# Wu-sm/Adversarial-Attacks-on-GAN-based-Image-Fusion

Hardware: AMD Instinct MI355X
Metric: attacked images/sec, PGD-20 L∞ ε=8/255 at 256², 1/2/4/8 MI355X (higher is better)
Workload: dtype f32; 1 GPU; PGD-20 L∞ eps=8/255 alpha=2/255 at 256², 128 images/GPU (BASELINE config #4 per-GPU share), RCCL all-gather of outputs when N>1; encoder=e4e, norm=linf, images_per_gpu=128, global_batch=128, size=256, pgd_steps=20, parallelism=dp1, dist_world_size=1, output_in_eps_ball_and_finite=True, fp32_arithmetic=fp32

## Files before the change

### adversarial-attacks-on-gan-based-image-fusion_amd/csrc/conv_common.h

```cpp
#pragma once
#include <algorithm>
#include <cstdlib>
#include <type_traits>

#include "mia_common.h"

namespace mia {

struct ConvGroup {
  const void* w;
  int kpad, kh, kw, pad_y, pad_x, ho, wo, ay, by, ax, bx, blk0, nbm, m;
  const void* w_split;
  int n_in, n_out, c_off;
};
constexpr int MIA_MAX_GROUPS = 16;

inline int pixels_clamped(int n, int h, int w) {
  const int64_t m = (int64_t)n * h * w;
  return m < 0 ? -1 : (m > 0x7fffffff ? 0x7fffffff : (int)m);
}

struct ConvK {
  mia_conv_args a;
  int stride, HT, WT, ystride, cout_mod, log2cin, n_first_max, ng, nblk, nbn;
// ... 338 lines not shown
            if (single) part[e] += c;
            else red_put(k, 0, pix, n * Cout + col + e, c);
          }
        }
        if (Y) {
          const size_t off = ((size_t)(n * k.HT + yo) * k.WT + xo) * k.ystride + cm;
          if (p.out_scale) {
            if (!single) load8f(p.out_scale + (size_t)n * k.cout_mod + cm, osc8);
#pragma unroll
            for (int e = 0; e < 8; ++e) v[e] *= osc8[e];
          }
          if (p.noise) {
            const float nz = p.noise_w * p.noise[yo * k.WT + xo];
#pragma unroll
            for (int e = 0; e < 8; ++e) v[e] += nz;
          }
          if (p.bias) {
#pragma unroll
            for (int e = 0; e < 8; ++e) v[e] += bias8[e];
          }
          float ma[8];
          if (TA) {
            float tt[8];
            load8<T>(TA + aoff, ma);
            load8<T>(TT + aoff, tt);
#pragma unroll
            for (int e = 0; e < 8; ++e) v[e] += p.tap_coef * (ma[e] - tt[e]);
          }
          if (MA) {
            if (MA != TA) load8<T>(MA + aoff, ma);
#pragma unroll
            for (int e = 0; e < 8; ++e) v[e] = ma[e] > 0.f ? v[e] : mslope8[e] * v[e];
          }
          if (prelu) {
#pragma unroll
            for (int e = 0; e < 8; ++e) v[e] = v[e] > 0.f ? v[e] : aslope8[e] * v[e];
          } else {
#pragma unroll
            for (int e = 0; e < 8; ++e) v[e] = apply_act(v[e], p.act_out);
          }
          if (p.accumulate) {
            float yo8[8];
            load8<T>(Y + off, yo8);
#pragma unroll
            for (int e = 0; e < 8; ++e) v[e] += yo8[e];
          }
          if (bab) {
            float dm8[8];
            load8f(p.bab_demod + (size_t)n * Cout + col, dm8);
            const float nz = p.bab_noise ? p.bab_noise_w * p.bab_noise[yo * k.WT + xo] : 0.f;
#pragma unroll
            for (int e = 0; e < 8; ++e) {
              const float gr = lrelu_s2_grad(xv[e]);
              const float gp = v[e] * gr;
              const float c = gp * (xv[e] * lrelu_s2_inv_grad(xv[e]) - nz - bbias8[e]);
              if (single) partq[e] += c;
              else red_put(k, 1, pix, n * Cout + col + e, c);
              v[e] = gp * dm8[e];
            }
          }
          if (p.csum) {
#pragma unroll
            for (int e = 0; e < 8; ++e) {
              if (single) pcs[e] += v[e];
              else red_put(k, 2, pix, n * Cout + col + e, v[e]);
            }
          }
          store8<T>(Y + off, v);
        }
      }
    }
    __syncthreads();
  }

  if (bab && single) {
#pragma unroll
    for (int e = 0; e < 8; ++e)
      for (int o = CPR; o < 64; o <<= 1) partq[e] += __shfl_xor(partq[e], o, 64);
    float* red = (float*)smem;
    if (worker && lane < CPR) {
#pragma unroll
      for (int e = 0; e < 8; ++e) red[wid * BN + lane * 8 + e] = partq[e];
    }
    __syncthreads();
    if (tid < BN && n0 + tid < Cout) {
      float s = 0.f;
#pragma unroll
      for (int w = 0; w < NW; ++w) s += red[w * BN + tid];
      red_put(k, 1, slot, n_single * Cout + n0 + tid, s);
    }
    __syncthreads();
  }
  if (p.csum && single) {
#pragma unroll
    for (int e = 0; e < 8; ++e)
      for (int o = CPR; o < 64; o <<= 1) pcs[e] += __shfl_xor(pcs[e], o, 64);
    float* red = (float*)smem;
    if (worker && lane < CPR) {
#pragma unroll
      for (int e = 0; e < 8; ++e) red[wid * BN + lane * 8 + e] = pcs[e];
    }
    __syncthreads();
    if (tid < BN && n0 + tid < Cout) {
      float s = 0.f;
#pragma unroll
      for (int w = 0; w < NW; ++w) s += red[w * BN + tid];
      red_put(k, 2, slot, n_single * Cout + n0 + tid, s);
    }
    __syncthreads();
  }
  if (p.sdot && single) {
#pragma unroll
    for (int e = 0; e < 8; ++e)
      for (int o = CPR; o < 64; o <<= 1) part[e] += __shfl_xor(part[e], o, 64);
    float* red = (float*)smem;
    if (worker && lane < CPR) {
#pragma unroll
      for (int e = 0; e < 8; ++e) red[wid * BN + lane * 8 + e] = part[e];
    }
    __syncthreads();
    if (tid < BN && n0 + tid < Cout) {
      float s = 0.f;
#pragma unroll
      for (int w = 0; w < NW; ++w) s += red[w * BN + tid];
      red_put(k, 0, slot, n_single * Cout + n0 + tid, s);
    }
  }
}

__device__ __forceinline__ void wait_vmcnt(int n) {
  switch (n) {
    case 0: asm volatile("s_waitcnt vmcnt(0)" ::: "memory"); break;
    case 1: asm volatile("s_waitcnt vmcnt(1)" ::: "memory"); break;
    case 2: asm volatile("s_waitcnt vmcnt(2)" ::: "memory"); break;
    case 3: asm volatile("s_waitcnt vmcnt(3)" ::: "memory"); break;
    case 4: asm volatile("s_waitcnt vmcnt(4)" ::: "memory"); break;
    case 5: asm volatile("s_waitcnt vmcnt(5)" ::: "memory"); break;
    case 6: asm volatile("s_waitcnt vmcnt(6)" ::: "memory"); break;
    case 7: asm volatile("s_waitcnt vmcnt(7)" ::: "memory"); break;
    case 8: asm volatile("s_waitcnt vmcnt(8)" ::: "memory"); break;
    case 9: asm volatile("s_waitcnt vmcnt(9)" ::: "memory"); break;
    case 10: asm volatile("s_waitcnt vmcnt(10)" ::: "memory"); break;
    case 11: asm volatile("s_waitcnt vmcnt(11)" ::: "memory"); break;
    case 12: asm volatile("s_waitcnt vmcnt(12)" ::: "memory"); break;
    case 13: asm volatile("s_waitcnt vmcnt(13)" ::: "memory"); break;
    case 14: asm volatile("s_waitcnt vmcnt(14)" ::: "memory"); break;
    case 15: asm volatile("s_waitcnt vmcnt(15)" ::: "memory"); break;
    default: asm volatile("s_waitcnt vmcnt(16)" ::: "memory"); break;
  }
}

bool conv_halo_x6_eligible(const ConvK& k, int dtype);
int launch_conv_halo_x6(ConvK& k, hipStream_t st);
bool conv_halo_eligible(const ConvK& k, int dtype);
int launch_conv_halo(ConvK& k, int dtype, hipStream_t st);
bool upconv_halo_eligible(int dtype, int R, int Cin, int Cout);
int launch_upconv_halo(const void* x, const void* w_up, const void* w_up_split, void* t, int N,
                       int R, int Cin, int Cout, int act_in, const float* style, int dtype,
                       hipStream_t st);
bool conv_wres_eligible(const ConvK& k, int dtype);
int launch_conv_wres(ConvK& k, int dtype, hipStream_t st);
bool conv_wres128_eligible(const ConvK& k, int dtype);
int launch_conv_wres128(ConvK& k, int dtype, hipStream_t st);
bool conv_wres32_eligible(const ConvK& k, int dtype);
int launch_conv_wres32(ConvK& k, int dtype, hipStream_t st);
bool conv_thin_eligible(const ConvK& k, int dtype);
bool conv_thin32_eligible(const ConvK& k, int dtype);
int launch_conv_thin32(ConvK& k, int dtype, hipStream_t st);
int launch_conv_thin(ConvK& k, int dtype, hipStream_t st);

}
```

### adversarial-attacks-on-gan-based-image-fusion_amd/csrc/conv_mfma.hip

```cpp
#include "conv_common.h"
#include <cstdio>
#include "halo_epilogue.h"

#ifndef MIA_F32_PRO_SMALLTILE
#define MIA_F32_PRO_SMALLTILE 128
#endif

namespace mia {

template <int PER>
__device__ __forceinline__ void wait_dma_steps(int steps) {
  static_assert(3 * PER <= 63, "vmcnt field");
  if (steps <= 0) asm volatile("s_waitcnt vmcnt(0)" ::: "memory");
  else if (steps == 1) asm volatile("s_waitcnt vmcnt(%0)" ::"n"(PER) : "memory");
  else if (steps == 2) asm volatile("s_waitcnt vmcnt(%0)" ::"n"(2 * PER) : "memory");
  else asm volatile("s_waitcnt vmcnt(%0)" ::"n"(3 * PER) : "memory");
}

template <typename T, int BM, int BN, bool X6B>
struct StageBytes {
  static constexpr int v = (BM + BN) * ROWB;
};
template <int BM, int BN>
struct StageBytes<float, BM, BN, true> {
// ... 311 lines not shown
    return -1;
  using namespace epi;
  const int f = epi_mask(k);
  switch (f) {
    case OSC | SDOT: case OSC | SDOT | ACC: case OSC | SDOT | BAB: case OSC | SDOT | ACC | BAB:
    case BIAS | PRELU:
    case BIAS: case ACC: case BIAS | ACC:
      return f;
    default:
      return -1;
  }
}

template <typename T, bool PRO, bool SMALLC>
static int launch_bn(ConvK& k, hipStream_t st) {
  int64_t m = 0;
  for (int g = 0; g < k.ng; ++g) m += k.g[g].m;
  if (k.a.Cout <= 64) {
    if constexpr (!PRO) {
      using namespace epi;
      switch (reg_epi_mask(k, sizeof(T))) {
        case OSC | SDOT: return launch_tile<T, Tile128x64, PRO, SMALLC, OSC | SDOT>(k, st);
        case OSC | SDOT | ACC:
          return launch_tile<T, Tile128x64, PRO, SMALLC, OSC | SDOT | ACC>(k, st);
        case OSC | SDOT | BAB:
          return launch_tile<T, Tile128x64, PRO, SMALLC, OSC | SDOT | BAB>(k, st);
        case OSC | SDOT | ACC | BAB:
          return launch_tile<T, Tile128x64, PRO, SMALLC, OSC | SDOT | ACC | BAB>(k, st);
        case BIAS | PRELU: return launch_tile<T, Tile128x64, PRO, SMALLC, BIAS | PRELU>(k, st);
        case BIAS: return launch_tile<T, Tile128x64, PRO, SMALLC, BIAS>(k, st);
        case ACC: return launch_tile<T, Tile128x64, PRO, SMALLC, ACC>(k, st);
        case BIAS | ACC: return launch_tile<T, Tile128x64, PRO, SMALLC, BIAS | ACC>(k, st);
        default: break;
      }
    }
    return launch_tile<T, Tile128x64, PRO, SMALLC>(k, st);
  }
  int64_t tiles = 0;
  for (int g = 0; g < k.ng; ++g) tiles += (k.g[g].m + 127) / 128;
  tiles *= (k.a.Cout + 127) / 128;
  const int64_t small_below = tune(T_CONV_SMALLTILE);
  if (sizeof(T) == 2 && tiles < small_below) return launch_tile<T, Tile64x64, PRO, SMALLC>(k, st);
  if (sizeof(T) == 4 && PRO && tiles < MIA_F32_PRO_SMALLTILE)
    return launch_tile<T, Tile64x64, PRO, SMALLC>(k, st);
  if constexpr (!SMALLC && !PRO) {
    using namespace epi;
    switch (reg_epi_mask(k, sizeof(T))) {
      case OSC | SDOT: return launch_tile<T, Tile128x128, PRO, SMALLC, OSC | SDOT>(k, st);
      case OSC | SDOT | ACC: return launch_tile<T, Tile128x128, PRO, SMALLC, OSC | SDOT | ACC>(k, st);
      case OSC | SDOT | BAB: return launch_tile<T, Tile128x128, PRO, SMALLC, OSC | SDOT | BAB>(k, st);
      case OSC | SDOT | ACC | BAB:
        return launch_tile<T, Tile128x128, PRO, SMALLC, OSC | SDOT | ACC | BAB>(k, st);
      case BIAS | PRELU: return launch_tile<T, Tile128x128, PRO, SMALLC, BIAS | PRELU>(k, st);
      case BIAS: return launch_tile<T, Tile128x128, PRO, SMALLC, BIAS>(k, st);
      case ACC: return launch_tile<T, Tile128x128, PRO, SMALLC, ACC>(k, st);
      case BIAS | ACC: return launch_tile<T, Tile128x128, PRO, SMALLC, BIAS | ACC>(k, st);
      default: break;
    }
  }
  return launch_tile<T, Tile128x128, PRO, SMALLC>(k, st);
}

static bool x6b_ok(const ConvK& k) {
#ifdef MIA_F32_NATIVE
  (void)k;
  return false;
#else
  if (tune(T_CONV_X6) == 0) return false;
  for (int g = 0; g < k.ng; ++g)
    if (!k.g[g].w_split) return false;
  return k.a.in_scale == nullptr && k.a.act_in == MIA_ACT_NONE && k.a.Cin >= 32 && k.a.Cout > 64;
#endif
}

template <typename T>
static int launch_conv(ConvK& k, hipStream_t st) {
  if constexpr (std::is_same<T, float>::value) {
    if (x6b_ok(k)) {
      using namespace epi;
      switch (reg_epi_mask(k, 4)) {
        case OSC | SDOT: return launch_tile<T, Tile128x128, false, false, OSC | SDOT, true>(k, st);
        case OSC | SDOT | ACC:
          return launch_tile<T, Tile128x128, false, false, OSC | SDOT | ACC, true>(k, st);
        case OSC | SDOT | BAB:
          return launch_tile<T, Tile128x128, false, false, OSC | SDOT | BAB, true>(k, st);
        case OSC | SDOT | ACC | BAB:
          return launch_tile<T, Tile128x128, false, false, OSC | SDOT | ACC | BAB, true>(k, st);
        case BIAS | PRELU: return launch_tile<T, Tile128x128, false, false, BIAS | PRELU, true>(k, st);
        case BIAS: return launch_tile<T, Tile128x128, false, false, BIAS, true>(k, st);
        case ACC: return launch_tile<T, Tile128x128, false, false, ACC, true>(k, st);
        case BIAS | ACC: return launch_tile<T, Tile128x128, false, false, BIAS | ACC, true>(k, st);
        default: break;
      }
      return launch_tile<T, Tile128x128, false, false, -2, true>(k, st);
    }
  }
  const bool pro = k.a.in_scale != nullptr || k.a.act_in != MIA_ACT_NONE;
  const bool small = k.a.Cin < ROWB / (int)sizeof(T);
  if (pro) return small ? launch_bn<T, true, true>(k, st) : launch_bn<T, true, false>(k, st);
  return small ? launch_bn<T, false, true>(k, st) : launch_bn<T, false, false>(k, st);
}

int conv_red_begin(ConvK& k, RedQ& r, int nslots, hipStream_t st, bool zero) {
  const mia_conv_args& a = k.a;
  const int count = a.N * a.Cout;
  const int rc = red_begin(r, a.sdot, a.bab_demod ? a.bab_q : nullptr, a.csum, nslots, count, st,
                           zero);
  k.red_part = r.part;
  k.red_nslots = nslots;
  k.red_count = count;
  return rc;
}

static int bk_for(int dtype) { return dtype == MIA_F32 ? 32 : 64; }

#ifndef MIA_UPCONV_EDGE_TRIM
#define MIA_UPCONV_EDGE_TRIM 1
#endif

static int kpad_for(int k, int dtype) {
  const int bk = bk_for(dtype);
  return (k + bk - 1) / bk * bk;
}

static int run_conv(ConvK& k, int dtype, hipStream_t st) {
  const mia_conv_args& a = k.a;
  MIA_CHECK_ARG(a.x, "x is required");
  MIA_CHECK_ARG(a.N > 0 && a.H > 0 && a.W > 0 && a.Cin > 0 && a.Cout > 0, "bad shape");
  MIA_CHECK_ARG(dtype == MIA_F32 || dtype == MIA_F16 || dtype == MIA_BF16, "bad dtype");
  const int vec = dtype == MIA_F32 ? 4 : 8;
  MIA_CHECK_ARG(a.Cin >= vec && (a.Cin & (a.Cin - 1)) == 0,
                "Cin must be a power of two ≥ the 16-byte vector");
  MIA_CHECK_ARG(a.Cout % 8 == 0, "Cout must be a multiple of 8");
  MIA_CHECK_ARG(!a.shuffle_out || (a.Cout % 32 == 0 && k.ng == 1), "shuffle_out: Cout % 32, 1 group");
  MIA_CHECK_ARG(!a.sdot || a.aux_x, "sdot needs aux_x");
  MIA_CHECK_ARG(!a.bab_demod || (a.aux_x && a.act_aux == MIA_ACT_NONE && a.bab_q && a.y &&
                                 !a.shuffle_out),
                "bab_demod needs aux_x (stored activations, act_aux NONE), bab_q and y");
  MIA_CHECK_ARG(!a.tap_a || a.tap_t, "tap_a needs tap_t");
  MIA_CHECK_ARG(a.act_out != MIA_ACT_PRELU || a.act_slope, "MIA_ACT_PRELU needs act_slope");
  MIA_CHECK_ARG(!a.csum || (a.y && !a.shuffle_out && k.ng == 1 &&
                             k.g[0].ho * k.g[0].wo == k.HT * k.WT),
                "csum needs y (un-shuffled), one group with an identity output placement");
  MIA_CHECK_ARG(!a.shuffle_out || !(a.tap_a || a.mask_a || a.sdot),
                "aux inputs need un-shuffled output");
  MIA_CHECK_ARG((int64_t)a.N * a.H * a.W * a.Cin < (1LL << 31), "input too large for 32-bit offsets");
  MIA_CHECK_ARG(a.in_scale == nullptr || a.Cin <= 2048, "modulated Cin ≤ 2048");
  MIA_CHECK_ARG(k.ng >= 1 && k.ng <= (k.batched ? MIA_MAX_GROUPS : 4), "1..4 groups (16 batched)");
  for (int g = 0; g < k.ng; ++g) {
    const ConvGroup& G = k.g[g];
    MIA_CHECK_ARG(G.w, "w is required");
    MIA_CHECK_ARG(G.kh >= 1 && G.kh <= 3 && G.kw >= 1 && G.kw <= 3, "taps 1..3");
    MIA_CHECK_ARG(G.kpad >= kpad_for(G.kh * G.kw * a.Cin, dtype) && G.kpad % bk_for(dtype) == 0,
                  "Kpad must be mia_conv_kpad()");
    MIA_CHECK_ARG(G.ho > 0 && G.wo > 0, "empty output grid");
    MIA_CHECK_ARG((int64_t)a.N * G.ho * G.wo < (1LL << 31), "too many pixels");
    MIA_CHECK_ARG(!(a.sdot || a.bab_demod) || (k.ng == 1 && G.ho * G.wo == k.HT * k.WT),
                  "sdot / bab need one group with an identity output placement");
    MIA_CHECK_ARG(G.ay * (G.ho - 1) + G.by < k.HT && G.ax * (G.wo - 1) + G.bx < k.WT &&
                      G.by >= 0 && G.bx >= 0,
                  "output placement outside the output grid");
  }
  int lc = 0;
  while ((1 << lc) < a.Cin) ++lc;
  k.log2cin = lc;
  int hw_min = 1 << 30;
  for (int g = 0; g < k.ng; ++g) hw_min = std::min(hw_min, k.g[g].ho * k.g[g].wo);
  k.n_first_max = std::min(a.N, (256 + hw_min - 1) / hw_min + 1);

  if (k.batched) {
    MIA_CHECK_ARG(!a.shuffle_out && !a.sdot && !a.bab_demod && !a.csum,
                  "batched groups: no shuffle_out / sdot / bab / csum");
    MIA_DISPATCH_DTYPE(dtype, T, return launch_conv<T>(k, st));
  }
  if (conv_thin_eligible(k, dtype)) return launch_conv_thin(k, dtype, st);
  if (conv_wres32_eligible(k, dtype)) return launch_conv_wres32(k, dtype, st);
  if (conv_thin32_eligible(k, dtype)) return launch_conv_thin32(k, dtype, st);
  if (conv_wres_eligible(k, dtype)) return launch_conv_wres(k, dtype, st);
  if (conv_wres128_eligible(k, dtype)) return launch_conv_wres128(k, dtype, st);
  if (conv_halo_x6_eligible(k, dtype)) return launch_conv_halo_x6(k, st);
  if (conv_halo_eligible(k, dtype)) return launch_conv_halo(k, dtype, st);
  MIA_DISPATCH_DTYPE(dtype, T, return launch_conv<T>(k, st));
  return MIA_OK;
}

}

using namespace mia;

extern "C" int mia_conv_kpad(int cin, int dtype) { return kpad_for(9 * cin, dtype); }

extern "C" int mia_conv3x3(const mia_conv_args* args, int dtype, void* stream) {
  MIA_CHECK_ARG(args != nullptr, "null args");
  const mia_conv_args& a = *args;
  MIA_CHECK_ARG(a.Kpad == kpad_for(9 * a.Cin, dtype), "Kpad must be mia_conv_kpad()");
  ConvK k = {};
  k.a = a;
  k.stride = 1;
  k.ng = 1;
  ConvGroup& G = k.g[0];
  G.w = a.w;
  G.w_split = a.w_split;
  G.kpad = a.Kpad;
  G.kh = G.kw = 3;
  G.pad_y = G.pad_x = 1;
  G.ho = a.H;
  G.wo = a.W;
  G.ay = G.ax = 1;
  G.m = pixels_clamped(a.N, a.H, a.W);
  k.HT = a.shuffle_out ? 2 * a.H : a.H;
  k.WT = a.shuffle_out ? 2 * a.W : a.W;
  k.cout_mod = a.shuffle_out ? a.Cout / 4 : a.Cout;
  k.ystride = a.y_cstride > 0 ? a.y_cstride : k.cout_mod;
  MIA_CHECK_ARG(k.ystride >= k.cout_mod, "y_cstride < Cout");
  return run_conv(k, dtype, (hipStream_t)stream);
}

extern "C" int mia_conv2d_kpad(int taps, int cin, int dtype) { return kpad_for(taps * cin, dtype); }

static int conv2d_impl(const mia_conv_args* args, int stride, const mia_conv_group* groups,
                       const mia_conv_batch* batch, int ngroups, int out_h, int out_w, int dtype,
                       void* stream, int ysplit = 0, int64_t yplane = 0);

extern "C" int mia_conv2d(const mia_conv_args* args, int stride, const mia_conv_group* groups,
                          int ngroups, int out_h, int out_w, int dtype, void* stream) {
  MIA_CHECK_ARG(ngroups >= 1 && ngroups <= 4, "1..4 groups");
  return conv2d_impl(args, stride, groups, nullptr, ngroups, out_h, out_w, dtype, stream);
}

extern "C" int mia_conv2d_batched(const mia_conv_args* args, int stride,
                                  const mia_conv_group* groups, const mia_conv_batch* batch,
                                  int ngroups, int out_h, int out_w, int dtype, void* stream) {
  MIA_CHECK_ARG(batch != nullptr, "null batch");
  MIA_CHECK_ARG(ngroups >= 1 && ngroups <= MIA_MAX_GROUPS, "1..16 groups");
  for (int g = 0; g < ngroups; ++g)
    MIA_CHECK_ARG(batch[g].n_in >= 0 && batch[g].n_out >= 0 && batch[g].c_off >= 0 &&
                      batch[g].c_off % 8 == 0,
                  "batch offsets must be ≥ 0 (c_off a multiple of 8)");
  return conv2d_impl(args, stride, groups, batch, ngroups, out_h, out_w, dtype, stream);
}

extern "C" int mia_conv2d_planes(const mia_conv_args* args, int stride,
                                 const mia_conv_group* groups, int out_h, int out_w,
                                 int plane_channels, int64_t plane_stride, int dtype,
                                 void* stream) {
  MIA_CHECK_ARG(args != nullptr && groups != nullptr, "null args");
  const mia_conv_args& a = *args;
  MIA_CHECK_ARG(stride == 2, "plane-split output: the stride-2 convs (generic tile) only");
  MIA_CHECK_ARG(plane_channels > 0 && plane_channels % 128 == 0 && a.Cout % plane_channels == 0,
                "plane_channels must be a multiple of 128 dividing Cout");
  MIA_CHECK_ARG(a.y_cstride == 0 || a.y_cstride == plane_channels, "y_cstride = plane_channels");
  MIA_CHECK_ARG(plane_stride >= (int64_t)a.N * out_h * out_w * plane_channels,
                "plane_stride < N·out_h·out_w·plane_channels");
  MIA_CHECK_ARG(a.y && !a.sdot && !a.bab_demod && !a.csum && !a.mask_a && !a.tap_a && !a.aux_x &&
                    !a.accumulate && !a.out_scale && !a.noise,
                "plane-split output: bias / act epilogues only");
  return conv2d_impl(args, stride, groups, nullptr, 1, out_h, out_w, dtype, stream,
                     plane_channels, plane_stride);
}

static int conv2d_impl(const mia_conv_args* args, int stride, const mia_conv_group* groups,
                       const mia_conv_batch* batch, int ngroups, int out_h, int out_w, int dtype,
                       void* stream, int ysplit, int64_t yplane) {
  MIA_CHECK_ARG(args != nullptr && groups != nullptr, "null args");
  MIA_CHECK_ARG(stride == 1 || stride == 2, "stride 1 or 2");
  MIA_CHECK_ARG(out_h > 0 && out_w > 0, "empty output");
  MIA_CHECK_ARG(!args->shuffle_out, "shuffle_out is a mia_conv3x3 feature");
  const mia_conv_args& a = *args;
  ConvK k = {};
  k.a = a;
  k.stride = stride;
  k.ng = ngroups;
  k.batched = batch != nullptr;
  k.HT = out_h;
  k.WT = out_w;
  k.cout_mod = a.Cout;
  k.ystride = a.y_cstride > 0 ? a.y_cstride : a.Cout;
  k.ysplit = ysplit;
  k.yplane = yplane;
  if (ysplit > 0) k.ystride = ysplit;
  MIA_CHECK_ARG(ysplit > 0 || k.ystride >= a.Cout, "y_cstride < Cout");
  for (int g = 0; g < ngroups; ++g) {
    const mia_conv_group& s = groups[g];
    ConvGroup& G = k.g[g];
    G.w = s.w;
    G.w_split = s.w_split;
    G.kh = s.kh;
    G.kw = s.kw;
    G.kpad = kpad_for(s.kh * s.kw * a.Cin, dtype);
    G.pad_y = s.pad_y;
    G.pad_x = s.pad_x;
    G.ho = s.ho;
    G.wo = s.wo;
    G.ay = s.ay;
    G.by = s.by;
    G.ax = s.ax;
    G.bx = s.bx;
    G.m = pixels_clamped(a.N, s.ho, s.wo);
    if (batch) {
      G.n_in = batch[g].n_in;
      G.n_out = batch[g].n_out;
      G.c_off = batch[g].c_off;
    }
  }
  return run_conv(k, dtype, (hipStream_t)stream);
}

extern "C" int mia_upconv_kpad(int cin, int phase, int dtype) {
  const int kh = 2 - (phase >> 1), kw = 2 - (phase & 1);
  return kpad_for(kh * kw * cin, dtype);
}

extern "C" int mia_upconv_fwd(const void* x, const void* const* w_phase, void* t_out, int N,
                              int R, int Cin, int Cout, int act_in, const float* style, int dtype,
                              void* stream) {
  MIA_CHECK_ARG(w_phase && t_out, "bad args");
  mia_conv_args a = {};
  a.x = x; a.y = t_out; a.N = N; a.H = R; a.W = R; a.Cin = Cin; a.Cout = Cout;
  a.act_in = act_in; a.in_scale = style;
  ConvK k = {};
  k.a = a;
  k.stride = 1;
  k.ng = 4;
  k.HT = k.WT = 2 * R + 1;
  k.cout_mod = Cout;
  k.ystride = Cout;
  for (int ph = 0; ph < 4; ++ph) {
    const int py = ph >> 1, px = ph & 1;
    ConvGroup& G = k.g[ph];
    G.w = w_phase[ph];
    G.kh = 2 - py;
    G.kw = 2 - px;
    G.kpad = kpad_for(G.kh * G.kw * Cin, dtype);
// ... 177 lines not shown
```

### adversarial-attacks-on-gan-based-image-fusion_amd/csrc/mia_common.h

```cpp
#pragma once
#include <hip/hip_runtime.h>
#include <stdint.h>
#include <string>

#include "../../include/miattack.h"

namespace mia {

typedef __attribute__((ext_vector_type(4))) float f32x4;
typedef __attribute__((ext_vector_type(8))) _Float16 f16x8;
typedef __attribute__((ext_vector_type(8))) __bf16 bf16x8;

template <typename T> struct Vec;
template <> struct Vec<float> { typedef f32x4 type; static constexpr int N = 4; };
template <> struct Vec<_Float16> { typedef f16x8 type; static constexpr int N = 8; };
template <> struct Vec<__bf16> { typedef bf16x8 type; static constexpr int N = 8; };

__device__ __forceinline__ float to_f(float v) { return v; }
__device__ __forceinline__ float to_f(_Float16 v) { return (float)v; }
__device__ __forceinline__ float to_f(__bf16 v) { return (float)v; }
template <typename T> __device__ __forceinline__ T from_f(float v);
template <> __device__ __forceinline__ float from_f<float>(float v) { return v; }
template <> __device__ __forceinline__ _Float16 from_f<_Float16>(float v) { return (_Float16)v; }
template <> __device__ __forceinline__ __bf16 from_f<__bf16>(float v) { return (__bf16)v; }

constexpr float SQRT2 = 1.41421356237309504880f;

__device__ __forceinline__ float lrelu_s2(float v) { return (v > 0.f ? v : 0.2f * v) * SQRT2; }
__device__ __forceinline__ float lrelu_s2_grad(float pre) { return pre > 0.f ? SQRT2 : 0.2f * SQRT2; }
__device__ __forceinline__ float lrelu_s2_inv_grad(float pre) {
  return pre > 0.f ? 0.70710678118654752f : 3.5355339059327376f;
}

#define MIA_DPP(v, ctrl) \
  __builtin_bit_cast(float, __builtin_amdgcn_mov_dpp(__builtin_bit_cast(int, (v)), (ctrl), 0xf, 0xf, false))
__device__ __forceinline__ void lds_handoff() {
  asm volatile("s_waitcnt lgkmcnt(0)\n\ts_barrier" ::: "memory");
}

__device__ __forceinline__ float row16_sum(float v) {
  v += MIA_DPP(v, 0xB1);
  v += MIA_DPP(v, 0x4E);
  v += MIA_DPP(v, 0x141);
  v += MIA_DPP(v, 0x140);
  return v;
}

__device__ __forceinline__ float wave_sum(float v) {
#pragma unroll
  for (int o = 32; o > 0; o >>= 1) v += __shfl_xor(v, o, 64);
  return v;
}

int set_error(const std::string& msg);
int check_launch(const char* what);

int device_cu_count();
int ensure_dyn_lds(const void* fn, int bytes);
int max_blocks_per_cu(const void* fn, int threads, size_t dyn_lds);

enum TuneKey {
  T_CONV_HALO,
  T_CONV_X6,
  T_HALO_EPI,
  T_X6_UNR,
  T_CONV_THIN,
  T_CONV_THIN32,
  T_CONV_WRES,
  T_CONV_REGEPI,
  T_CONV_SMALLTILE,
  T_S2DG_X6,
  T_S2DG_HALO,
  T_UPCONV_X6,
  T_UPCONV_HALO,
  T_CONV_WRES32,
  T_HALO_C64,
  T_X6_64S,
  T_UPCONV_X6S,
  T_CONV_WRES128,
  T_X6_STAGGER,
  T_NKEYS
};
int tune(TuneKey key);

struct RedQ {
  float* dst[3];
  float* part;
  int nslots, count;
};
float* red_scratch(hipStream_t st, size_t bytes);
int red_begin(RedQ& r, float* d0, float* d1, float* d2, int nslots, int count, hipStream_t st,
              bool zero = false);
int red_finish(const RedQ& r, hipStream_t st);

__device__ __forceinline__ void red_store(float* part, int nslots, int count, int q, int slot,
                                          int i, float v) {
  part[((size_t)q * nslots + slot) * count + i] = v;
}

}

#define MIA_DISPATCH_DTYPE(dtype, T, ...)                                   \
  switch (dtype) {                                                          \
    case MIA_F32: { typedef float T; __VA_ARGS__; break; }                  \
    case MIA_F16: { typedef _Float16 T; __VA_ARGS__; break; }               \
    case MIA_BF16: { typedef __bf16 T; __VA_ARGS__; break; }                \
    default: return mia::set_error("unsupported dtype");                    \
  }

#define MIA_CHECK_ARG(cond, msg) \
  do { if (!(cond)) return mia::set_error(std::string(__func__) + ": " + (msg)); } while (0)
```

### adversarial-attacks-on-gan-based-image-fusion_amd/csrc/reduce.hip

```cpp
#include <algorithm>
#include <cstdlib>
#include <cstring>
#include <mutex>
#include <unordered_map>
#include <vector>

#include "mia_common.h"

namespace mia {

namespace {
struct Scratch {
  float* p = nullptr;
  size_t bytes = 0;
};
std::mutex g_mu;
std::unordered_map<hipStream_t, Scratch> g_scratch;
}

namespace {
struct TuneDef {
  const char* name;
  int value;
};
TuneDef g_tune[T_NKEYS] = {
    {"MIA_CONV_HALO", 1}, {"MIA_CONV_X6", 1},       {"MIA_HALO_EPI", 1},    {"MIA_X6_UNR", 2},
    {"MIA_CONV_THIN", 1}, {"MIA_CONV_THIN32", 1},   {"MIA_CONV_WRES", 1},
    {"MIA_CONV_REGEPI", 1},   {"MIA_CONV_SMALLTILE", 512},
    {"MIA_S2DG_X6", 1},   {"MIA_S2DG_HALO", 1},     {"MIA_UPCONV_X6", 1},   {"MIA_UPCONV_HALO", 1},
    {"MIA_CONV_WRES32", 1},
    {"MIA_HALO_C64", 1},  {"MIA_X6_64S", 1},
    {"MIA_UPCONV_X6S", 1}, {"MIA_CONV_WRES128", 1}, {"MIA_X6_STAGGER", -1}};
std::once_flag g_tune_once;
void tune_init() {
  for (auto& d : g_tune) {
    if (&d == &g_tune[T_X6_STAGGER]) continue;
    const char* e = getenv(d.name);
    if (e && *e) d.value = atoi(e);
  }
}
}

int tune(TuneKey key) {
  std::call_once(g_tune_once, tune_init);
  return g_tune[key].value;
}

namespace {
std::mutex g_dev_mu;
std::unordered_map<int, int> g_ncu;
std::unordered_map<const void*, std::vector<int>> g_lds_set;
int current_device() {
  int dev = 0;
  (void)hipGetDevice(&dev);
  return dev;
}
}

int device_cu_count() {
  const int dev = current_device();
  std::lock_guard<std::mutex> lock(g_dev_mu);
  auto it = g_ncu.find(dev);
  if (it != g_ncu.end()) return it->second;
  int ncu = 0;
  if (hipDeviceGetAttribute(&ncu, hipDeviceAttributeMultiprocessorCount, dev) != hipSuccess ||
      ncu <= 0)
    ncu = 256;
  g_ncu[dev] = ncu;
  return ncu;
}

int ensure_dyn_lds(const void* fn, int bytes) {
  const int dev = current_device();
  std::lock_guard<std::mutex> lock(g_dev_mu);
  std::vector<int>& done = g_lds_set[fn];
  if (std::find(done.begin(), done.end(), dev) != done.end()) return MIA_OK;
  if (hipFuncSetAttribute(fn, hipFuncAttributeMaxDynamicSharedMemorySize, bytes) != hipSuccess)
    return set_error("hipFuncSetAttribute(MaxDynamicSharedMemorySize) failed");
  done.push_back(dev);
  return MIA_OK;
}

int max_blocks_per_cu(const void* fn, int threads, size_t dyn_lds) {
  static std::unordered_map<const void*, std::unordered_map<int, int>> cache;
  const int dev = current_device();
  std::lock_guard<std::mutex> lock(g_dev_mu);
  auto& per_dev = cache[fn];
  auto it = per_dev.find(dev);
  if (it != per_dev.end()) return it->second;
  int occ = 0;
  if (hipOccupancyMaxActiveBlocksPerMultiprocessor(&occ, fn, threads, dyn_lds) != hipSuccess ||
      occ < 1)
    occ = 1;
  per_dev[dev] = occ;
  return occ;
}

float* red_scratch(hipStream_t st, size_t bytes) {
  std::lock_guard<std::mutex> lock(g_mu);
  Scratch& s = g_scratch[st];
  if (s.bytes >= bytes) return s.p;
  if (s.p) {
    if (hipStreamSynchronize(st) != hipSuccess || hipFree(s.p) != hipSuccess) return nullptr;
    s.p = nullptr;
    s.bytes = 0;
  }
  size_t want = bytes < (1u << 20) ? (1u << 20) : bytes;
  want = want + want / 4;
  void* p = nullptr;
  if (hipMalloc(&p, want) != hipSuccess) return nullptr;
  s.p = (float*)p;
  s.bytes = want;
  return s.p;
}

constexpr int RED_CHUNK = 64;
static inline int red_nchunks(int nslots) { return nslots <= 2 * RED_CHUNK ? 1 : (nslots + RED_CHUNK - 1) / RED_CHUNK; }

int red_begin(RedQ& r, float* d0, float* d1, float* d2, int nslots, int count, hipStream_t st,
              bool zero) {
  r.dst[0] = d0;
  r.dst[1] = d1;
  r.dst[2] = d2;
  r.nslots = nslots;
  r.count = count;
  r.part = nullptr;
  if (!d0 && !d1 && !d2) return MIA_OK;
  if (nslots < 1 || count < 1) return set_error("red_begin: empty reduction");
  const int nch = red_nchunks(nslots);
  const size_t part_bytes = (size_t)3 * nslots * count * sizeof(float);
  const size_t bytes = part_bytes + (nch > 1 ? (size_t)3 * nch * count * sizeof(float) : 0);
  r.part = red_scratch(st, bytes);
  if (!r.part) return set_error("red_begin: scratch allocation failed");
  if (zero && hipMemsetAsync(r.part, 0, part_bytes, st) != hipSuccess)
    return set_error("red_begin: memset failed");
  return MIA_OK;
}

__device__ __forceinline__ float ordered_sum(const float* __restrict__ src, int n, int stride) {
  float s = 0.f;
  int k = 0;
  for (; k + 8 <= n; k += 8) {
    float t[8];
#pragma unroll
    for (int u = 0; u < 8; ++u) t[u] = src[(size_t)(k + u) * stride];
#pragma unroll
    for (int u = 0; u < 8; ++u) s += t[u];
  }
  for (; k < n; ++k) s += src[(size_t)k * stride];
  return s;
}

__global__ __launch_bounds__(256) void red_finish_kernel(const float* __restrict__ part,
                                                         float* d0, float* d1, float* d2,
                                                         int nslots, int count) {
  const int q = blockIdx.y;
  float* dst = q == 0 ? d0 : (q == 1 ? d1 : d2);
  if (!dst) return;
  const int i = blockIdx.x * 256 + threadIdx.x;
  if (i >= count) return;
  const float* src = part + (size_t)q * nslots * count + i;
  dst[i] += ordered_sum(src, nslots, count);
}

__global__ __launch_bounds__(256) void red_chunk_kernel(const float* __restrict__ part,
                                                        float* __restrict__ tmp, int has0,
                                                        int has1, int has2, int nslots,
                                                        int count) {
  const int q = blockIdx.z, c = blockIdx.y;
  if (!(q == 0 ? has0 : (q == 1 ? has1 : has2))) return;
  const int i = blockIdx.x * 256 + threadIdx.x;
  if (i >= count) return;
  const int k0 = c * RED_CHUNK, k1 = min(k0 + RED_CHUNK, nslots);
  const float* src = part + ((size_t)q * nslots + k0) * count + i;
  tmp[((size_t)q * gridDim.y + c) * count + i] = ordered_sum(src, k1 - k0, count);
}

int red_finish(const RedQ& r, hipStream_t st) {
  if (!r.part) return MIA_OK;
  const int nch = red_nchunks(r.nslots);
  if (nch == 1) {
    hipLaunchKernelGGL(red_finish_kernel, dim3((r.count + 255) / 256, 3), dim3(256), 0, st,
                       r.part, r.dst[0], r.dst[1], r.dst[2], r.nslots, r.count);
    return check_launch("red_finish");
  }
  float* tmp = r.part + (size_t)3 * r.nslots * r.count;
  hipLaunchKernelGGL(red_chunk_kernel, dim3((r.count + 255) / 256, nch, 3), dim3(256), 0, st,
                     r.part, tmp, r.dst[0] != nullptr, r.dst[1] != nullptr, r.dst[2] != nullptr,
                     r.nslots, r.count);
// ... 73 lines not shown
```

Baseline: 17.26 attacked images/s.

## Add halo-tiled stride-2 3x3 conv kernel with split-precision MFMA

Adds a dedicated stride-2 3x3 convolution kernel that loads an input halo tile (even/odd column split) into LDS once per channel block, converts it to hi/lo split format, and reuses it across all nine taps, while double-buffering weight tiles. It is inserted into the dispatch ahead of the generic halo and implicit-GEMM paths for eligible f32 stride-2 layers. The aim is to cut redundant global loads of input pixels for downsampling convolutions in the encoder. The trade-off is a full barrier and conversion pass per channel block and extra LDS use, which allows only two blocks per CU.

Measured after the change: 17.31 attacked images/s, median of 6. About the same (+0.3%).

```diff
diff --git a/adversarial-attacks-on-gan-based-image-fusion_amd/csrc/conv_common.h b/adversarial-attacks-on-gan-based-image-fusion_amd/csrc/conv_common.h
--- a/adversarial-attacks-on-gan-based-image-fusion_amd/csrc/conv_common.h
+++ b/adversarial-attacks-on-gan-based-image-fusion_amd/csrc/conv_common.h
@@ -514,6 +514,8 @@
 
 bool conv_halo_x6_eligible(const ConvK& k, int dtype);
 int launch_conv_halo_x6(ConvK& k, hipStream_t st);
+bool conv_halo_s2_eligible(const ConvK& k, int dtype);
+int launch_conv_halo_s2(ConvK& k, hipStream_t st);
 bool conv_halo_eligible(const ConvK& k, int dtype);
 int launch_conv_halo(ConvK& k, int dtype, hipStream_t st);
 bool upconv_halo_eligible(int dtype, int R, int Cin, int Cout);
diff --git a/adversarial-attacks-on-gan-based-image-fusion_amd/csrc/conv_halo_s2.hip b/adversarial-attacks-on-gan-based-image-fusion_amd/csrc/conv_halo_s2.hip
--- /dev/null
+++ b/adversarial-attacks-on-gan-based-image-fusion_amd/csrc/conv_halo_s2.hip
@@ -0,0 +1,262 @@
+#include "conv_common.h"
+#include "halo_epilogue.h"
+
+namespace mia {
+
+struct HaloS2 {
+  static constexpr int PH = 8, PW = 16, NW = 4, NT = 64 * NW;
+  static constexpr int WM = 2, WN = 2, FM = 4, FN = 4;
+  static constexpr int BM = PH * PW, BN = 128, BK = 16;
+  static constexpr int HH = 2 * PH + 1, HSIDE = 2 * PW + 1, HROWS = HH * HSIDE;
+  static constexpr int NEVEN = PW + 1;
+  static constexpr int HROWB = 64, LROWB = 32;
+  static constexpr int HPIECES = (HROWS + 15) / 16;
+  static constexpr int HBUF = HPIECES * 1024, LBUF = HROWS * LROWB;
+  static constexpr int BHM = BN * HROWB, BL = BN * LROWB, BSTAGE = BHM + BL;
+  static constexpr int B_HM_INS = BN / 16 / NW, B_L_INS = BN / 32 / NW;
+  static constexpr int H_INS = HPIECES / NW;
+  static constexpr int EROWS = 128, ES = BN + 4;
+  static constexpr int LDS = HBUF + LBUF + 2 * BSTAGE;
+  static_assert(WM * FM * 16 == BM && WN * FN * 16 == BN, "");
+  static_assert(H_INS * NW == HPIECES && B_HM_INS * 16 * NW == BN && B_L_INS * 32 * NW == BN, "");
+  static_assert(LBUF % 16 == 0 && LDS <= 80 * 1024, "two blocks per CU");
+};
+
+template <>
+struct EpiChunk<HaloS2> {
+  static constexpr int FMC = 2;
+};
+
+__device__ __forceinline__ int fsw64(int row) { return ((row >> 2) & 1) << 1; }
+__device__ __forceinline__ int lsw32(int row) { return ((row >> 3) & 1) << 1; }
+
+template <int EPI>
+__global__ __launch_bounds__(HaloS2::NT, 2) void conv_halo_s2_kernel(const ConvK k) {
+  typedef HaloS2 TL;
+  constexpr int FM = TL::FM, FN = TL::FN, NT = TL::NT, BN = TL::BN, BK = TL::BK;
+  constexpr int HSIDE = TL::HSIDE, HROWS = TL::HROWS, HROWB = TL::HROWB, LROWB = TL::LROWB;
+  constexpr int H_INS = TL::H_INS, B_HM_INS = TL::B_HM_INS, B_L_INS = TL::B_L_INS;
+  constexpr int BSTAGE = TL::BSTAGE;
+
+  extern __shared__ __attribute__((aligned(16))) char smem[];
+  char* const hbuf = smem;
+  char* const lbuf = smem + TL::HBUF;
+  char* const bring = lbuf + TL::LBUF;
+
+  const mia_conv_args& p = k.a;
+  const int tid = threadIdx.x, lane = tid & 63;
+  const int wid = __builtin_amdgcn_readfirstlane(tid >> 6);
+  const int wm = wid / TL::WN, wn = wid % TL::WN;
+  const ConvGroup G = k.g[0];
+  const int H = p.H, W = p.W, Cin = p.Cin, Cout = p.Cout, Kpad = G.kpad;
+  const int Ho = G.ho, Wo = G.wo;
+  const int bl = xcd_remap(blockIdx.x, k.nblk);
+  const int mt = bl / k.nbn, n0 = (bl % k.nbn) * BN;
+  const int ptx = Wo / TL::PW, pty = Ho / TL::PH;
+  const int x0 = (mt % ptx) * TL::PW;
+  const int y0 = ((mt / ptx) % pty) * TL::PH;
+  const int n = mt / (ptx * pty);
+
+  const float* __restrict__ X = (const float*)p.x;
+  const unsigned* __restrict__ Whm = (const unsigned*)G.w_split;
+  const __bf16* __restrict__ Wl = (const __bf16*)(Whm + (size_t)Cout * Kpad);
+  const char* zero = (const char*)g_zero16;
+
+  const char* wsrc[B_HM_INS + B_L_INS];
+#pragma unroll
+  for (int j = 0; j < B_HM_INS + B_L_INS; ++j) {
+    if (j < B_HM_INS) {
+      const int row = (wid * B_HM_INS + j) * 16 + (lane >> 2);
+      const int c = min(n0 + row, Cout - 1);
+      wsrc[j] = (const char*)(Whm + (size_t)c * Kpad + ((lane & 3) ^ fsw64(row)) * 4);
+    } else {
+      const int row = (wid * B_L_INS + j - B_HM_INS) * 32 + (lane >> 1);
+      const int c = min(n0 + row, Cout - 1);
+      wsrc[j] = (const char*)(Wl + (size_t)c * Kpad + ((lane & 1) ^ (lsw32(row) >> 1)) * 8);
+    }
+  }
+  const char* hsrc[H_INS];
+#pragma unroll
+  for (int j = 0; j < H_INS; ++j) {
+    hsrc[j] = nullptr;
+    const int hr = (wid + TL::NW * j) * 16 + (lane >> 2);
+    const int hy = hr / HSIDE, sl = hr - hy * HSIDE;
+    const int hx = sl < TL::NEVEN ? 2 * sl : 2 * (sl - TL::NEVEN) + 1;
+    const int y = 2 * y0 + hy - G.pad_y, x = 2 * x0 + hx - G.pad_x;
+    if (hr < HROWS && y >= 0 && y < H && x >= 0 && x < W)
+      hsrc[j] = (const char*)(X + ((size_t)(n * H + y) * W + x) * Cin + ((lane & 3) ^ fsw64(hr)) * 4);
+  }
+  const int ncb = Cin / BK, nk = 9 * ncb;
+
+  auto issue_b = [&](int s, int st) {
+    const int cb = s / 9, t = s - (s / 9) * 9;
+    const size_t koff = (size_t)t * Cin + cb * BK;
+    char* dst = bring + st * BSTAGE;
+#pragma unroll
+    for (int j = 0; j < B_HM_INS; ++j)
+      __builtin_amdgcn_global_load_lds((gptr_t)(wsrc[j] + koff * 4),
+                                       (lptr_t)(dst + (wid * B_HM_INS + j) * 1024), 16, 0, 0);
+#pragma unroll
+    for (int j = 0; j < B_L_INS; ++j)
+      __builtin_amdgcn_global_load_lds((gptr_t)(wsrc[B_HM_INS + j] + koff * 2),
+                                       (lptr_t)(dst + TL::BHM + (wid * B_L_INS + j) * 1024), 16,
+                                       0, 0);
+  };
+  auto issue_halo = [&](int cb) {
+#pragma unroll
+    for (int j = 0; j < H_INS; ++j) {
+      const char* a = hsrc[j] ? hsrc[j] + (size_t)cb * BK * 4 : zero;
+      __builtin_amdgcn_global_load_lds((gptr_t)a, (lptr_t)(hbuf + (wid + TL::NW * j) * 1024), 16,
+                                       0, 0);
+    }
+  };
+  auto convert = [&]() {
+    for (int c = tid; c < HROWS * 4; c += NT) {
+      const int hr = c >> 2, pc = c & 3, lc = pc ^ fsw64(hr);
+      const f32x4 v = *(const f32x4*)(hbuf + hr * HROWB + pc * 16);
+      u32x4 hm;
+      u32x2 lo;
+      split_quad(v, hm, lo);
+      *(u32x4*)(hbuf + hr * HROWB + pc * 16) = hm;
+      *(u32x2*)(lbuf + hr * LROWB + ((lc ^ lsw32(hr)) << 3)) = lo;
+    }
+  };
+
+  issue_halo(0);
+  issue_b(0, 0);
+  asm volatile("s_waitcnt vmcnt(0)" ::: "memory");
+  __syncthreads();
+  convert();
+  __syncthreads();
+
+  f32x4 acc[FM][FN];
+#pragma unroll
+  for (int i = 0; i < FM; ++i)
+#pragma unroll
+    for (int j = 0; j < FN; ++j) acc[i][j] = f32x4{0.f, 0.f, 0.f, 0.f};
+
+  const int frow = lane & 15, fq = lane >> 4;
+  int oh[2 * FM + 1][3], ol[2 * FM + 1][3];
+#pragma unroll
+  for (int q = 0; q < 2 * FM + 1; ++q)
+#pragma unroll
+    for (int c = 0; c < 3; ++c) {
+      const int cs = c == 0 ? 0 : (c == 1 ? TL::NEVEN : 1);
+      const int hr = (2 * wm * FM + q) * HSIDE + cs + frow;
+      int vh = hr * HROWB + ((fq ^ fsw64(hr)) << 4), vl = hr * LROWB + ((fq ^ lsw32(hr)) << 3);
+      asm volatile("" : "+v"(vh), "+v"(vl));
+      oh[q][c] = vh;
+      ol[q][c] = vl;
+    }
+  int ob[FN], obl[FN];
+#pragma unroll
+  for (int j = 0; j < FN; ++j) {
+    const int row = wn * FN * 16 + 16 * j + frow;
+    ob[j] = row * HROWB + ((fq ^ fsw64(row)) << 4);
+    obl[j] = TL::BHM + row * LROWB + ((fq ^ lsw32(row)) << 3);
+  }
+  int st = 0;
+  for (int cb = 0; cb < ncb; ++cb) {
+#pragma unroll
+    for (int t = 0; t < 9; ++t) {
+      const int s = cb * 9 + t;
+      const int dy = t / 3, dx = t % 3;
+      const char* sb = bring + st * BSTAGE;
+      if (s + 1 < nk) issue_b(s + 1, st ^ 1);
+      u32x4 ahm[FM], bhm[FN];
+      u32x2 al[FM], blo[FN];
+#pragma unroll
+      for (int i = 0; i < FM; ++i) {
+        ahm[i] = *(const u32x4*)(hbuf + oh[2 * i + dy][dx]);
+        al[i] = *(const u32x2*)(lbuf + ol[2 * i + dy][dx]);
+      }
+#pragma unroll
+      for (int j = 0; j < FN; ++j) {
+        bhm[j] = *(const u32x4*)(sb + ob[j]);
+        blo[j] = *(const u32x2*)(sb + obl[j]);
+      }
+      __builtin_amdgcn_s_setprio(1);
+#pragma unroll
+      for (int i = 0; i < FM; ++i)
+#pragma unroll
+        for (int j = 0; j < FN; ++j)
+          acc[i][j] = EPI != -2 ? mfma_x6(bhm[j], blo[j], ahm[i], al[i], acc[i][j])
+                                : mfma_x6(ahm[i], al[i], bhm[j], blo[j], acc[i][j]);
+      __builtin_amdgcn_s_setprio(0);
+      asm volatile("s_waitcnt vmcnt(0)" ::: "memory");
+      lds_handoff();
+      __builtin_amdgcn_sched_barrier(0);
+      st ^= 1;
+    }
+    if (cb + 1 < ncb) {
+      issue_halo(cb + 1);
+      asm volatile("s_waitcnt vmcnt(0)" ::: "memory");
+      __syncthreads();
+      convert();
+      __syncthreads();
+    }
+  }
+  if constexpr (EPI >= 0) {
+    halo_epilogue_f<float, TL, EPI>(k, acc, n, y0, x0, n0, wm, wn, lane, Ho, Wo, nullptr,
+                                    k.prered ? (float*)smem : nullptr, TL::WM, TL::BN);
+  } else {
+    __syncthreads();
+    const int img_row = n * Ho + y0;
+    conv_epilogue<float, TL>(k, G, acc, smem, n0, true, n, [=](int r) {
+      return (img_row + (r >> 4)) * Wo + x0 + (r & 15);
+    }, (y0 / TL::PH) * (Wo / TL::PW) + x0 / TL::PW);
+  }
+}
+
+template <int EPI>
+static int launch_s2_(ConvK& k, hipStream_t st) {
+  typedef HaloS2 TL;
+  const ConvGroup& G = k.g[0];
+  k.nbn = (k.a.Cout + TL::BN - 1) / TL::BN;
+  k.nblk = k.a.N * (G.ho / TL::PH) * (G.wo / TL::PW) * k.nbn;
+  size_t lds = TL::LDS;
+  lds = std::max(lds, (size_t)TL::EROWS * TL::ES * 4);
+  lds = std::max(lds, (size_t)TL::NW * TL::BN * 4);
+  auto fn = conv_halo_s2_kernel<EPI>;
+  if (const int rc = ensure_dyn_lds((const void*)fn, 80 * 1024); rc != MIA_OK) return rc;
+  k.prered = EPI >= 0 && (EPI & epi::CSUM);
+  k.red_px = 0;
+  const int nslots = EPI >= 0 ? halo_red_slots(G.ho, G.wo, TL::FM, TL::WM, k.prered)
+                              : (G.ho / TL::PH) * (G.wo / TL::PW);
+  RedQ r;
+  int rc = conv_red_begin(k, r, nslots, st);
+  if (rc != MIA_OK) return rc;
+  hipLaunchKernelGGL(fn, dim3(k.nblk), dim3(TL::NT), lds, st, k);
+  rc = check_launch("conv_halo_s2");
+  return rc != MIA_OK ? rc : red_finish(r, st);
+}
+
+bool conv_halo_s2_eligible(const ConvK& k, int dtype) {
+#ifdef MIA_F32_NATIVE
+  (void)k;
+  (void)dtype;
+  return false;
+#endif
+  if (tune(T_CONV_X6) == 0 || tune(T_CONV_HALO_S2) == 0) return false;
+  const mia_conv_args& a = k.a;
+  const ConvGroup& G = k.g[0];
+  return dtype == MIA_F32 && G.w_split != nullptr && k.ng == 1 && !k.batched && k.stride == 2 &&
+         G.kh == 3 && G.kw == 3 && G.pad_y == G.pad_x && (G.pad_y == 0 || G.pad_y == 1) &&
+         G.ay == 1 && G.ax == 1 && G.by == 0 && G.bx == 0 && !a.shuffle_out &&
+         G.ho % HaloS2::PH == 0 && G.wo % HaloS2::PW == 0 && k.HT == G.ho && k.WT == G.wo &&
+         G.kpad >= 9 * a.Cin && a.in_scale == nullptr && a.act_in == MIA_ACT_NONE &&
+         a.Cin % 32 == 0 && a.Cout > 64;
+}
+
+int launch_conv_halo_s2(ConvK& k, hipStream_t st) {
+  using namespace epi;
+  switch (epi_mask(k)) {
+    case BIAS | PRELU: return launch_s2_<BIAS | PRELU>(k, st);
+    case BIAS: return launch_s2_<BIAS>(k, st);
+    case BIAS | ACC: return launch_s2_<BIAS | ACC>(k, st);
+    case OSC | SDOT | ACC | BAB: return launch_s2_<OSC | SDOT | ACC | BAB>(k, st);
+    default: return launch_s2_<-2>(k, st);
+  }
+}
+
+}
diff --git a/adversarial-attacks-on-gan-based-image-fusion_amd/csrc/conv_mfma.hip b/adversarial-attacks-on-gan-based-image-fusion_amd/csrc/conv_mfma.hip
--- a/adversarial-attacks-on-gan-based-image-fusion_amd/csrc/conv_mfma.hip
+++ b/adversarial-attacks-on-gan-based-image-fusion_amd/csrc/conv_mfma.hip
@@ -487,7 +487,7 @@
     MIA_CHECK_ARG(G.w, "w is required");
     MIA_CHECK_ARG(G.kh >= 1 && G.kh <= 3 && G.kw >= 1 && G.kw <= 3, "taps 1..3");
     MIA_CHECK_ARG(G.kpad >= kpad_for(G.kh * G.kw * a.Cin, dtype) && G.kpad % bk_for(dtype) == 0,
-                  "Kpad must be mia_conv_kpad()");
+                  "group kpad must be a multiple of the K-step covering kh·kw·Cin");
     MIA_CHECK_ARG(G.ho > 0 && G.wo > 0, "empty output grid");
     MIA_CHECK_ARG((int64_t)a.N * G.ho * G.wo < (1LL << 31), "too many pixels");
     MIA_CHECK_ARG(!(a.sdot || a.bab_demod) || (k.ng == 1 && G.ho * G.wo == k.HT * k.WT),
@@ -514,6 +514,7 @@
   if (conv_wres_eligible(k, dtype)) return launch_conv_wres(k, dtype, st);
   if (conv_wres128_eligible(k, dtype)) return launch_conv_wres128(k, dtype, st);
   if (conv_halo_x6_eligible(k, dtype)) return launch_conv_halo_x6(k, st);
+  if (conv_halo_s2_eligible(k, dtype)) return launch_conv_halo_s2(k, st);
   if (conv_halo_eligible(k, dtype)) return launch_conv_halo(k, dtype, st);
   MIA_DISPATCH_DTYPE(dtype, T, return launch_conv<T>(k, st));
   return MIA_OK;
diff --git a/adversarial-attacks-on-gan-based-image-fusion_amd/csrc/mia_common.h b/adversarial-attacks-on-gan-based-image-fusion_amd/csrc/mia_common.h
--- a/adversarial-attacks-on-gan-based-image-fusion_amd/csrc/mia_common.h
+++ b/adversarial-attacks-on-gan-based-image-fusion_amd/csrc/mia_common.h
@@ -79,6 +79,7 @@
   T_UPCONV_X6S,
   T_CONV_WRES128,
   T_X6_STAGGER,
+  T_CONV_HALO_S2,
   T_NKEYS
 };
 int tune(TuneKey key);
diff --git a/adversarial-attacks-on-gan-based-image-fusion_amd/csrc/reduce.hip b/adversarial-attacks-on-gan-based-image-fusion_amd/csrc/reduce.hip
--- a/adversarial-attacks-on-gan-based-image-fusion_amd/csrc/reduce.hip
+++ b/adversarial-attacks-on-gan-based-image-fusion_amd/csrc/reduce.hip
@@ -30,11 +30,12 @@
     {"MIA_S2DG_X6", 1},   {"MIA_S2DG_HALO", 1},     {"MIA_UPCONV_X6", 1},   {"MIA_UPCONV_HALO", 1},
     {"MIA_CONV_WRES32", 1},
     {"MIA_HALO_C64", 1},  {"MIA_X6_64S", 1},
-    {"MIA_UPCONV_X6S", 1}, {"MIA_CONV_WRES128", 1}, {"MIA_X6_STAGGER", -1}};
+    {"MIA_UPCONV_X6S", 1}, {"MIA_CONV_WRES128", 1}, {"MIA_X6_STAGGER", -1},
+    {"MIA_CONV_HALO_S2", 1}};
 std::once_flag g_tune_once;
 void tune_init() {
   for (auto& d : g_tune) {
-    if (&d == &g_tune[T_X6_STAGGER]) continue;
+    if (&d == &g_tune[T_X6_STAGGER] || &d == &g_tune[T_CONV_HALO_S2]) continue;
     const char* e = getenv(d.name);
     if (e && *e) d.value = atoi(e);
   }
```
